# WeChatCV/WeDetect

Measured on AMD Instinct MI355X. Metric: images/s at 640x640 (WeDetect-Base image tower + 80-class similarity + top-k/NMS), higher is better.
Workload: dtype f32-equivalent: fp32 operands carried as fp16 hi+lo pairs, 3 fp16-MFMA passes per product, fp32 accumulate (fp16x3); similarity GEMM, dwconv, LN, post-process native f32

## Files before the change

### wedetect_amd/build.py

```python
from __future__ import annotations

import os
import subprocess
import sys

HERE = os.path.dirname(os.path.abspath(__file__))
ROOT = os.path.dirname(HERE)
CSRC = os.path.join(HERE, "csrc")
LIB = os.path.join(HERE, "libwedetect_hip.so")
SOURCES = ["abi.hip", "conv_gemm.hip", "similarity_grouped.hip", "split_gemm.hip", "split_gemm_pre.hip", "split_gemm_p8.hip", "split_gemm_p4.hip", "split_gemm_conv.hip", "split_gemm_conv3.hip", "split_gemm_mlp.hip", "split_gemm_mlpw.hip", "probe.hip", "stem.hip", "elementwise.hip", "preprocess.hip", "text.hip", "bricks.hip", "evaluate.hip", "det_eval.hip", "postprocess.hip"]
HIPCC = os.environ.get("HIPCC", "/opt/rocm/bin/hipcc")
FLAGS = ["--offload-arch=gfx950", "-O3", "-std=c++17", "-fPIC", "-Wall", "-Wno-unused-function", "-Wno-inline-asm",
         "-I", os.path.join(ROOT, "include"), "-I", CSRC]
for _d in os.environ.get("WD_EXTRA_DEFINES", "").split():
    FLAGS.append("-D" + _d)
if os.environ.get("WD_DEBUG_ABLATIONS") == "1":
    FLAGS.append("-DWD_DEBUG_ABLATIONS")


def _headers():
    return [os.path.join(CSRC, f) for f in os.listdir(CSRC) if f.endswith(".h")] + [os.path.join(ROOT, "include", "wedetect_hip.h")]


def source_hash() -> str:
    import hashlib
    h = hashlib.sha256()
    files = sorted(os.path.join(CSRC, f) for f in os.listdir(CSRC) if f.endswith((".hip", ".h")))
    for f in files + [os.path.join(ROOT, "include", "wedetect_hip.h")]:
        h.update(os.path.basename(f).encode())
        h.update(open(f, "rb").read())
    return h.hexdigest()


NO_SCRATCH = {"stem.hip": ["stem_fused_kernel"], "split_gemm_mlpw.hip": ["fused_mlp_wide_kernel"],
              "split_gemm_mlp.hip": ["fused_mlp128_kernel"], "split_gemm_p8.hip": ["split_gemm_p8_kernel"],
              "split_gemm_p4.hip": ["split_gemm_p4_kernel"], "split_gemm_conv.hip": ["split_conv_pp_kernel"],
              "split_gemm_conv3.hip": ["split_conv3_kernel", "split_conv3w_kernel"],
              "split_gemm_pre.hip": ["split_gemm_pingpong_kernel", "split_gemm_glds_kernel"],
              "elementwise.hip": ["dwconv7_dma_kernel", "dwconv7_ln_reg4_dma_kernel"],
              "similarity_grouped.hip": ["similarity_grouped_kernel"]}
ASM_VMEM_SOURCES = {"split_gemm_mlpw.hip": ["fused_mlp_wide_kernel"], "split_gemm_mlp.hip": [], "split_gemm_p8.hip": [],
                    "split_gemm_p4.hip": [], "split_gemm_pre.hip": [], "split_gemm_conv.hip": [], "split_gemm_conv3.hip": [], "stem.hip": [], "elementwise.hip": [], "similarity_grouped.hip": []}


ASM_DS_READ_SOURCES = {"split_gemm_conv3.hip": ["split_conv3w_kernel"]}


def check_isa(src: str, verbose: bool = True) -> None:
    asm = _obj(src).replace(".o", ".s")
    cmd = [HIPCC, *[f for f in FLAGS if f != "-fPIC"], "-S", "--cuda-device-only", os.path.join(CSRC, src), "-o", asm]
    subprocess.check_call(cmd, stderr=subprocess.DEVNULL)
    scripts = os.path.join(ROOT, "scripts")
    r = subprocess.run([sys.executable, os.path.join(scripts, "check_sgpr_vmem_hazard.py"), asm], capture_output=True, text=True)
    if r.returncode != 0:
        raise RuntimeError(f"SGPR -> VMEM hazard in the ISA of {src}:\n{r.stdout[-2000:]}")
    syms = ASM_VMEM_SOURCES[src]
    if syms:
        r = subprocess.run([sys.executable, os.path.join(scripts, "check_asm_loads.py"), asm, *syms], capture_output=True, text=True)
        if r.returncode != 0:
            raise RuntimeError(f"pending asm load touched in the ISA of {src}:\n{r.stdout[-2000:]}")
    if src in ASM_DS_READ_SOURCES:
        r = subprocess.run([sys.executable, os.path.join(scripts, "check_asm_ds_reads.py"), asm, *ASM_DS_READ_SOURCES[src]], capture_output=True, text=True)
        if r.returncode != 0:
            raise RuntimeError(f"pending asm ds_read touched in the ISA of {src}:\n{r.stdout[-2000:]}")
    if src in NO_SCRATCH:
        import re
        meta = open(asm).read()
        meta = meta[meta.index("amdhsa.kernels"):] if "amdhsa.kernels" in meta else ""
        seen = set()
        for blk in meta.split("- .agpr_count")[1:]:
            name = re.search(r"\.name:\s+(\S+)", blk).group(1)
            scratch = int(re.search(r"\.private_segment_fixed_size:\s+(\d+)", blk).group(1))
            for k in NO_SCRATCH[src]:
                if k in name:
                    seen.add(k)
                    if scratch != 0:
                        raise RuntimeError(f"{src}: kernel {name} uses {scratch} bytes of scratch — its counted vmcnt waits assume none")
        missing = [k for k in NO_SCRATCH[src] if k not in seen]
        if missing:
            raise RuntimeError(f"{src}: NO_SCRATCH names no kernel of this source: {missing}")
    os.remove(asm)
    if verbose:
        print(f"ISA checks passed: {src}", flush=True)


def _obj(src: str) -> str:
    return os.path.join(CSRC, src.replace(".hip", ".o"))


def _obj_stale(src: str) -> bool:
    obj = _obj(src)
    if not os.path.exists(obj):
        return True
    t = os.path.getmtime(obj)
    return any(os.path.getmtime(d) > t for d in [os.path.join(CSRC, src)] + _headers())


def _stale() -> bool:
    if not os.path.exists(LIB):
        return True
    t = os.path.getmtime(LIB)
    return any(_obj_stale(s) or os.path.getmtime(_obj(s)) > t for s in SOURCES)


def build(force: bool = False, verbose: bool = True) -> str:
    if not force and not _stale():
        return LIB
    procs = []
    for src in SOURCES:
        if not force and not _obj_stale(src):
            continue
        cmd = [HIPCC, *FLAGS, "-c", os.path.join(CSRC, src), "-o", _obj(src)]
        if verbose:
            print(" ".join(cmd), flush=True)
        procs.append((src, subprocess.Popen(cmd)))
    import concurrent.futures as cf
    with cf.ThreadPoolExecutor(max_workers=4) as ex:
        checks = [ex.submit(check_isa, src, verbose) for src, _ in procs if src in ASM_VMEM_SOURCES]
        for src, p in procs:
            if p.wait() != 0:
                raise RuntimeError(f"hipcc failed on {src}")
        for c in checks:
            c.result()
    cmd = [HIPCC, "--offload-arch=gfx950", "-shared", "-fPIC", *[_obj(s) for s in SOURCES], "-o", LIB]
    if verbose:
        print(" ".join(cmd), flush=True)
    subprocess.check_call(cmd)
    return LIB


if __name__ == "__main__":
    print(build(force="--force" in sys.argv))
```

### wedetect_amd/csrc/split_gemm_mlpw.hip

```cpp
#include <stdlib.h>
#include "split_epi_oct.h"
#include "split_mlp_epi.h"

namespace {

template <int C>
struct MW {
  static constexpr int H = 4 * C, BM = 128, HC = 128, NCH = H / HC;
  static constexpr int KT = 64, NKT = C / KT;
  static constexpr int XSLOT = BM * 256, NSLOT = 3;
  static constexpr int HOFF = NSLOT * XSLOT;
  static constexpr int LDS = HOFF + BM * 512;
  static constexpr int TN2 = C / 128;
  static constexpr int S1 = C / 16, S2 = H / 16;
  static_assert(C % 128 == 0 && NKT >= 2 && LDS <= 160 * 1024, "shape");
  static_assert(4 * 32 * EPI_LDT * 4 <= HOFF, "the epilogue patches reuse the ring");
};

struct MwArgs {
  const unsigned char* a;
  const unsigned char* w1;
  const unsigned char* w2;
  const float* b1;
  const float* b2;
  float* x;
  unsigned* range_flag;
  int m;
  float unscale1, unscale2, hid_scale;
  unsigned* flag;
  float* park;
  int nblk;
  const float* ln_stats;
  const float* ln_u;
};

#define MW_OPAQUE(p) asm volatile("" : "+s"(p))
template <bool SAFE>
__device__ __forceinline__ void mw_dma(unsigned lds_addr, unsigned voff, const unsigned char* base) {
  if constexpr (SAFE)
    asm volatile("s_mov_b32 m0, %0\n\ts_nop 4\n\tglobal_load_lds_dwordx4 %1, %2" ::"s"(lds_addr), "v"(voff), "s"(base) : "memory", "m0");
  else
    asm volatile("s_mov_b32 m0, %0\n\ts_nop 0\n\tglobal_load_lds_dwordx4 %1, %2" ::"s"(lds_addr), "v"(voff), "s"(base) : "memory", "m0");
}

#ifdef MW_EXPERIMENT_LGKM
#define MW_LGKM0 "s_waitcnt lgkmcnt(0)"
#else
#define MW_LGKM0 ""
#endif
#define MW_BARRIER()                          \
  do {                                        \
    __builtin_amdgcn_sched_barrier(0);        \
    asm volatile(MW_LGKM0 ::: "memory");      \
    __builtin_amdgcn_s_barrier();             \
    asm volatile("" ::: "memory");            \
    __builtin_amdgcn_sched_barrier(0);        \
  } while (0)

template <bool SAFE>
__device__ __forceinline__ void mw_wload(h8& hi, h8& lo, unsigned lane16, const unsigned char* base) {
  if constexpr (SAFE)
    asm volatile("s_nop 4\n\tglobal_load_dwordx4 %0, %2, %3\n\tglobal_load_dwordx4 %1, %2, %3 offset:1024"
                 : "=&v"(hi), "=&v"(lo) : "v"(lane16), "s"(base) : "memory");
  else
    asm volatile("global_load_dwordx4 %0, %2, %3\n\tglobal_load_dwordx4 %1, %2, %3 offset:1024"
                 : "=&v"(hi), "=&v"(lo) : "v"(lane16), "s"(base) : "memory");
}
template <bool SAFE>
__device__ __forceinline__ void mw_bload(f32x4& d, unsigned voff, const float* base) {
  if constexpr (SAFE)
    asm volatile("s_nop 4\n\tglobal_load_dwordx4 %0, %1, %2" : "=&v"(d) : "v"(voff), "s"(base) : "memory");
  else
    asm volatile("global_load_dwordx4 %0, %1, %2" : "=&v"(d) : "v"(voff), "s"(base) : "memory");
}
#define MW_WAIT8_(N, A0, A1, A2, A3, A4, A5, A6, A7) \
  asm volatile("s_waitcnt vmcnt(" #N ")" : "+v"(A0), "+v"(A1), "+v"(A2), "+v"(A3), "+v"(A4), "+v"(A5), "+v"(A6), "+v"(A7) :: "memory")
#ifdef MW_EXPERIMENT_ALL0
#define MW_WAIT8(N, ...) MW_WAIT8_(0, __VA_ARGS__)
#else
#define MW_WAIT8(N, ...) MW_WAIT8_(N, __VA_ARGS__)
#endif

template <int C, int ABL = 0, bool PERSIST = false, bool FOLD = false>
__global__ void __launch_bounds__(256) fused_mlp_wide_kernel(const MwArgs q) {
  using P = MW<C>;
  constexpr int TN2 = P::TN2, NKT = P::NKT;
  static_assert(NKT % 2 == 0 && NKT >= 4, "K tiles alternate between two W1 fragment buffers");
  extern __shared__ __attribute__((aligned(16))) unsigned char smem_raw[];
  const int t = threadIdx.x, lane = t & 63;
  const int wave = __builtin_amdgcn_readfirstlane(t >> 6);
  int first_blk, seg_o, last_blk, seg_e;
  if (PERSIST) {
    const int b = blockIdx.x, xcd = b & 7, slot = b >> 3, per = gridDim.x >> 3;
    const long long t0 = (long long)q.nblk * xcd / 8, t1 = (long long)q.nblk * (xcd + 1) / 8;
    const long long units = (t1 - t0) * P::NCH;
    const long long u0 = t0 * P::NCH + units * slot / per, u1 = t0 * P::NCH + units * (slot + 1) / per;
    first_blk = (int)(u0 / P::NCH); seg_o = (int)(u0 - (long long)first_blk * P::NCH);
    last_blk = (int)(u1 / P::NCH); seg_e = (int)(u1 - (long long)last_blk * P::NCH);
  } else {
    int tile = blockIdx.x;
    const int nwg = gridDim.x, xcd = tile & 7, idx = tile >> 3;
    const int qq = nwg >> 3, r = nwg & 7;
    tile = (xcd < r ? xcd * (qq + 1) : r * (qq + 1) + (xcd - r) * qq) + idx;
    first_blk = tile; seg_o = 0; last_blk = tile + 1; seg_e = 0;
  }
  const int has_head = seg_e > 0, has_tail = seg_o > 0;
  const int full0 = first_blk + has_tail, nfull = last_blk - full0;
  const int nseg = has_head + nfull + has_tail;
  unsigned lds0 = (unsigned)(size_t)(__attribute__((address_space(3))) unsigned char*)smem_raw;

  unsigned la[4];
#pragma unroll
  for (int c = 0; c < 4; ++c) la[c] = (unsigned)(lane >> 4) * (unsigned)(C * 4) + (unsigned)((((lane & 15) ^ (4 * c + (lane >> 4))) & 15) << 4);
  const unsigned char* arow = q.a;
  auto issue_x = [&](int kt, int slot) {
    if (ABL & 2) return;
#pragma unroll
    for (int i = 0; i < 8; ++i) {
      const int g = wave * 8 + i;
      mw_dma<PERSIST>(lds0 + slot * P::XSLOT + g * 1024, la[i & 3], arow + (size_t)(4 * g) * (C * 4) + kt * 256);
    }
  };

  const int r = lane & 31, hsel = lane >> 5, f = r & 15;
  const int xb = r * 256 + (((2 * hsel) ^ f) << 4);
  const int hb = r * 512 + (((2 * hsel) ^ f) << 4);
  const unsigned char* hbuf = smem_raw + P::HOFF;

  const unsigned lane16 = (unsigned)lane * 16u;
  const unsigned char* w1w_ = q.w1 + (size_t)wave * (P::S1 * 2048);
  const unsigned char* w2w_ = q.w2 + (size_t)(TN2 * wave) * (P::S2 * 2048);
  const unsigned char *w1w = w1w_, *w2w = w2w_;
  const unsigned bvoff = (unsigned)hsel * 16u;
  const float* b1p = q.b1 + wave * 32;
  const float* u1p = FOLD ? q.ln_u + wave * 32 : nullptr;

  using I0 = std::integral_constant<int, 0>;
  using I1 = std::integral_constant<int, 1>;

  for (int sg = 0; sg < nseg; ++sg) {
  const bool is_head = has_head && sg == 0;
  const bool is_tail = has_tail && sg == nseg - 1;
  const int blk = is_head ? last_blk : (is_tail ? first_blk : full0 + sg - has_head);
  const int c0 = is_tail ? seg_o : 0, c1 = is_head ? seg_e : P::NCH;
  const int m0 = blk * P::BM;
  arow = q.a + (size_t)m0 * (C * 4);
  MW_BARRIER();

  f32x16 out[4][TN2];
  if (PERSIST && is_tail) {
    const int prev = blockIdx.x - 8;
    if (t == 0) {
      while (__hip_atomic_load(q.flag + prev, __ATOMIC_RELAXED, __HIP_MEMORY_SCOPE_AGENT) != 1u) __builtin_amdgcn_s_sleep(8);
      __builtin_amdgcn_fence(__ATOMIC_ACQUIRE, "agent");
    }
    __syncthreads();
    const unsigned char* sb = reinterpret_cast<const unsigned char*>(q.park) + (size_t)prev * (4 * TN2 * 4 * 4096);
    const unsigned toff = (unsigned)t * 16u;
#pragma unroll
    for (int i = 0; i < 4; ++i) {
      f32x4 v[TN2][4];
#pragma unroll
      for (int jn = 0; jn < TN2; ++jn)
#pragma unroll
        for (int g = 0; g < 4; ++g) {
          MW_OPAQUE(sb);
          v[jn][g] = *reinterpret_cast<const f32x4*>(sb + toff);
          sb += 4096;
        }
#pragma unroll
      for (int jn = 0; jn < TN2; ++jn)
#pragma unroll
        for (int g = 0; g < 4; ++g) {
          out[i][jn][4 * g] = v[jn][g][0]; out[i][jn][4 * g + 1] = v[jn][g][1]; out[i][jn][4 * g + 2] = v[jn][g][2]; out[i][jn][4 * g + 3] = v[jn][g][3];
        }
      __builtin_amdgcn_sched_barrier(0);
#pragma unroll
      for (int jn = 0; jn < TN2; ++jn) asm volatile("" : "+a"(out[i][jn]));
      __builtin_amdgcn_sched_barrier(0);
    }
    asm volatile("s_waitcnt vmcnt(0)" ::: "memory");
    __syncthreads();
    if (t == 0) __hip_atomic_store(q.flag + prev, 0u, __ATOMIC_RELAXED, __HIP_MEMORY_SCOPE_AGENT);
  } else {
#pragma unroll
    for (int i = 0; i < 4; ++i)
#pragma unroll
      for (int jn = 0; jn < TN2; ++jn)
#pragma unroll
        for (int e = 0; e < 16; ++e) out[i][jn][e] = 0.0f;
  }

  h8 wh[2][4], wl[2][4];
  h8 vh[2][TN2], vl[2][TN2];
  f32x4 bq[4];
  f32x4 uq[4] = {};
  typedef float f32x2_ __attribute__((ext_vector_type(2)));
  f32x2_ st[4] = {};

  auto load_w1_tile = [&](int j, int kt, int buf) {
    if ((ABL & 8) && (j > c0 || kt > 1)) return;
    const unsigned char* b = w1w + (size_t)(4 * j) * (P::S1 * 2048) + kt * 8192;
#pragma unroll
    for (int s = 0; s < 4; ++s) mw_wload<PERSIST>(wh[buf][s], wl[buf][s], lane16, b + s * 2048);
  };
  auto load_w2_step = [&](int S, int buf) {
    if ((ABL & 8) && S > 1) return;
    const unsigned char* b = w2w + (size_t)S * 2048;
#pragma unroll
    for (int jn = 0; jn < TN2; ++jn) mw_wload<PERSIST>(vh[buf][jn], vl[buf][jn], lane16, b + (size_t)jn * (P::S2 * 2048));
  };
  auto load_bias = [&](int j) {
    const float* b = b1p + j * P::HC;
#pragma unroll
    for (int g = 0; g < 4; ++g) mw_bload<PERSIST>(bq[g], bvoff, b + 8 * g);
    if constexpr (FOLD) {
      const float* u = u1p + j * P::HC;
#pragma unroll
      for (int g = 0; g < 4; ++g) mw_bload<PERSIST>(uq[g], bvoff, u + 8 * g);
    }
  };

  MW_OPAQUE(arow); MW_OPAQUE(w1w); MW_OPAQUE(w2w); MW_OPAQUE(b1p); MW_OPAQUE(lds0);
  issue_x(0, 0);
  issue_x(1, 1);
  load_w1_tile(c0, 0, 0);
  load_w1_tile(c0, 1, 1);
  load_bias(c0);
  if constexpr (FOLD) {
    const float* sp = q.ln_stats + 2 * (size_t)m0;
    MW_OPAQUE(sp);
#pragma unroll
    for (int i = 0; i < 4; ++i) {
      const unsigned so = (unsigned)(32 * i + r) * 8u;
      if constexpr (PERSIST) asm volatile("s_nop 4\n\tglobal_load_dwordx2 %0, %1, %2" : "=&v"(st[i]) : "v"(so), "s"(sp) : "memory");
      else asm volatile("global_load_dwordx2 %0, %1, %2" : "=&v"(st[i]) : "v"(so), "s"(sp) : "memory");
    }
    asm volatile("s_waitcnt vmcnt(0)" : "+v"(st[0]), "+v"(st[1]), "+v"(st[2]), "+v"(st[3]) :: "memory");
  } else {
    asm volatile("s_waitcnt vmcnt(0)" ::: "memory");
  }

  for (int j = c0; j < c1; ++j) {
    const int jn1 = j + 1 < c1 ? j + 1 : j;
    MW_OPAQUE(arow); MW_OPAQUE(w1w); MW_OPAQUE(w2w); MW_OPAQUE(b1p); MW_OPAQUE(lds0);
    f32x16 g1[4];
#pragma unroll
    for (int i = 0; i < 4; ++i)
#pragma unroll
      for (int e = 0; e < 16; ++e) g1[i][e] = 0.0f;

    auto ktile = [&](auto kt_c, auto buf_c, int slot) {
      constexpr int KT_ = decltype(kt_c)::value, BUF = decltype(buf_c)::value;
      if (!(ABL & 2)) {
#ifdef MW_EXPERIMENT_TILE_WAIT
        MW_WAIT8(MW_EXPERIMENT_TILE_WAIT, wh[BUF][0], wl[BUF][0], wh[BUF][1], wl[BUF][1], wh[BUF][2], wl[BUF][2], wh[BUF][3], wl[BUF][3]);
#else
        if constexpr (KT_ == 0 && TN2 == 2 && FOLD) MW_WAIT8(20, wh[BUF][0], wl[BUF][0], wh[BUF][1], wl[BUF][1], wh[BUF][2], wl[BUF][2], wh[BUF][3], wl[BUF][3]);
        else if constexpr (KT_ == 0 && TN2 == 2) MW_WAIT8(16, wh[BUF][0], wl[BUF][0], wh[BUF][1], wl[BUF][1], wh[BUF][2], wl[BUF][2], wh[BUF][3], wl[BUF][3]);
        else if constexpr (KT_ <= 1 && FOLD) MW_WAIT8(24, wh[BUF][0], wl[BUF][0], wh[BUF][1], wl[BUF][1], wh[BUF][2], wl[BUF][2], wh[BUF][3], wl[BUF][3]);
        else if constexpr (KT_ <= 1) MW_WAIT8(20, wh[BUF][0], wl[BUF][0], wh[BUF][1], wl[BUF][1], wh[BUF][2], wl[BUF][2], wh[BUF][3], wl[BUF][3]);
        else if constexpr (KT_ == NKT - 1) MW_WAIT8(8, wh[BUF][0], wl[BUF][0], wh[BUF][1], wl[BUF][1], wh[BUF][2], wl[BUF][2], wh[BUF][3], wl[BUF][3]);
        else MW_WAIT8(16, wh[BUF][0], wl[BUF][0], wh[BUF][1], wl[BUF][1], wh[BUF][2], wl[BUF][2], wh[BUF][3], wl[BUF][3]);
#endif
      }
      if (!(ABL & 4)) MW_BARRIER();
      {
        int s2 = slot + 2;
        if (s2 >= P::NSLOT) s2 -= P::NSLOT;
        issue_x(KT_ + 2 < NKT ? KT_ + 2 : KT_ + 2 - NKT, s2);
      }
      const unsigned char* xs = smem_raw + slot * P::XSLOT;
      const unsigned char* wnext = w1w + (size_t)(4 * j) * (P::S1 * 2048) + (KT_ + 2) * 8192;
      h8 xh[2][4], xl[2][4];
      auto read_x = [&](int ks, h8 (&fh)[4], h8 (&fl)[4]) {
#pragma unroll
        for (int i = 0; i < 4; ++i) {
          fh[i] = *reinterpret_cast<const h8*>(xs + i * 8192 + (xb ^ (ks * 64)));
          fl[i] = *reinterpret_cast<const h8*>(xs + i * 8192 + (xb ^ (ks * 64 + 16)));
        }
      };
      read_x(0, xh[0], xl[0]);
      __builtin_amdgcn_sched_barrier(0);
#pragma unroll
      for (int ks = 0; ks < 4; ++ks) {
        const int cb = ks & 1;
        if (ks < 3) read_x(ks + 1, xh[cb ^ 1], xl[cb ^ 1]);
#pragma unroll
        for (int i = 0; i < 4; ++i) g1[i] = __builtin_amdgcn_mfma_f32_32x32x16_f16(wl[BUF][ks], xh[cb][i], g1[i], 0, 0, 0);
#pragma unroll
        for (int i = 0; i < 4; ++i) g1[i] = __builtin_amdgcn_mfma_f32_32x32x16_f16(wh[BUF][ks], xl[cb][i], g1[i], 0, 0, 0);
#pragma unroll
        for (int i = 0; i < 4; ++i) g1[i] = __builtin_amdgcn_mfma_f32_32x32x16_f16(wh[BUF][ks], xh[cb][i], g1[i], 0, 0, 0);
        if (ks < 3) {
#pragma unroll
          for (int u = 0; u < 8; ++u) {
            __builtin_amdgcn_sched_group_barrier(0x008, 1, 0);
            __builtin_amdgcn_sched_group_barrier(0x100, 1, 0);
          }
          __builtin_amdgcn_sched_group_barrier(0x008, 4, 0);
        }
        __builtin_amdgcn_sched_barrier(0);
        if constexpr (KT_ + 2 < NKT) {
          if (!(ABL & 8)) mw_wload<PERSIST>(wh[BUF][ks], wl[BUF][ks], lane16, wnext + ks * 2048);
        }
      }
    };
    {
      int slot = 0;
      slot = ((j - c0) * (NKT % P::NSLOT)) % P::NSLOT;
      auto adv = [&]() { slot = slot + 1 == P::NSLOT ? 0 : slot + 1; };
      ktile(std::integral_constant<int, 0>{}, I0{}, slot); adv();
      ktile(std::integral_constant<int, 1>{}, I1{}, slot); adv();
      ktile(std::integral_constant<int, 2>{}, I0{}, slot); adv();
      ktile(std::integral_constant<int, 3>{}, I1{}, slot); adv();
      if constexpr (NKT == 8) {
        ktile(std::integral_constant<int, 4>{}, I0{}, slot); adv();
        ktile(std::integral_constant<int, 5>{}, I1{}, slot); adv();
        ktile(std::integral_constant<int, 6>{}, I0{}, slot); adv();
        ktile(std::integral_constant<int, 7>{}, I1{}, slot); adv();
      }
    }

    load_w2_step(8 * j, 0);
    load_w2_step(8 * j + 1, 1);
#ifdef MW_EXPERIMENT_ALL0
    asm volatile("s_waitcnt vmcnt(0)" : "+v"(bq[0]), "+v"(bq[1]), "+v"(bq[2]), "+v"(bq[3]) :: "memory");
#else
    asm volatile("s_waitcnt vmcnt(48)" : "+v"(bq[0]), "+v"(bq[1]), "+v"(bq[2]), "+v"(bq[3]) :: "memory");
#endif
    if constexpr (FOLD) asm volatile("" : "+v"(uq[0]), "+v"(uq[1]), "+v"(uq[2]), "+v"(uq[3]));

#pragma unroll
    for (int i = 0; i < 4; ++i) {
      u32x2 hi[4], lo[4];
#pragma unroll
      for (int g = 0; g < 4; ++g) {
        if (ABL & 1) {
          hi[g] = u32x2{__builtin_bit_cast(unsigned, g1[i][4 * g]), __builtin_bit_cast(unsigned, g1[i][4 * g + 1])};
          lo[g] = u32x2{__builtin_bit_cast(unsigned, g1[i][4 * g + 2]), __builtin_bit_cast(unsigned, g1[i][4 * g + 3])};
        } else {
          const f32x4 v = {g1[i][4 * g], g1[i][4 * g + 1], g1[i][4 * g + 2], g1[i][4 * g + 3]};
          f32x4 o;
#pragma unroll
          for (int e = 0; e < 4; ++e) {
            if constexpr (FOLD) o[e] = wd_gelu(fmaf(st[i][1], fmaf(-st[i][0], uq[g][e], v[e] * q.unscale1), bq[g][e]));
            else o[e] = wd_gelu(fmaf(v[e], q.unscale1, bq[g][e]));
          }
          if (q.hid_scale != 1.0f) o = o * q.hid_scale;
          split4(o, hi[g], lo[g]);
        }
      }
#pragma unroll
      for (int s = 0; s < 2; ++s) {
        h8 fh8, fl8;
        mc_epi_swap(hi, lo, s, fh8, fl8);
        const int grp = 4 * wave + 2 * s + hsel;
        unsigned char* hp = smem_raw + P::HOFF + (32 * i + r) * 512;
        *reinterpret_cast<h8*>(hp + (((2 * grp) ^ f) << 4)) = fh8;
        *reinterpret_cast<h8*>(hp + (((2 * grp + 1) ^ f) << 4)) = fl8;
      }
    }
    asm volatile("s_waitcnt lgkmcnt(0)" ::: "memory");
    MW_BARRIER();

    h8 hh[2][4], hl[2][4];
    auto read_h = [&](int ks, h8 (&fh)[4], h8 (&fl)[4]) {
#pragma unroll
      for (int i = 0; i < 4; ++i) {
        fh[i] = *reinterpret_cast<const h8*>(hbuf + i * 16384 + (hb ^ (ks * 64)));
        fl[i] = *reinterpret_cast<const h8*>(hbuf + i * 16384 + (hb ^ (ks * 64 + 16)));
      }
    };
    auto g2step = [&](auto ks_c, auto buf_c) {
      constexpr int KS = decltype(ks_c)::value, BUF = decltype(buf_c)::value;
      static_assert(TN2 == 4 || TN2 == 2, "wait operand lists");
      if constexpr (TN2 == 4) {
#define MW_W2WAIT(N) MW_WAIT8(N, vh[BUF][0], vl[BUF][0], vh[BUF][1], vl[BUF][1], vh[BUF][2], vl[BUF][2], vh[BUF][3], vl[BUF][3])
        if constexpr (KS <= 4) MW_W2WAIT(8); else if constexpr (KS == 5) MW_W2WAIT(16); else if constexpr (KS == 6) MW_W2WAIT(24); else if constexpr (FOLD) MW_W2WAIT(16); else MW_W2WAIT(12);
#undef MW_W2WAIT
      } else {
#ifdef MW_EXPERIMENT_ALL0
#define MW_W2WAIT(N) asm volatile("s_waitcnt vmcnt(0)" : "+v"(vh[BUF][0]), "+v"(vl[BUF][0]), "+v"(vh[BUF][1]), "+v"(vl[BUF][1]) :: "memory")
#else
#define MW_W2WAIT(N) asm volatile("s_waitcnt vmcnt(" #N ")" : "+v"(vh[BUF][0]), "+v"(vl[BUF][0]), "+v"(vh[BUF][1]), "+v"(vl[BUF][1]) :: "memory")
#endif
        if constexpr (KS <= 4) MW_W2WAIT(4); else if constexpr (KS == 5) MW_W2WAIT(12); else if constexpr (KS == 6) MW_W2WAIT(20); else if constexpr (FOLD) MW_W2WAIT(16); else MW_W2WAIT(12);
#undef MW_W2WAIT
      }
      if constexpr (KS == 0) {
        read_h(0, hh[0], hl[0]);
        __builtin_amdgcn_sched_barrier(0);
      }
      if constexpr (KS < 7) read_h(KS + 1, hh[BUF ^ 1], hl[BUF ^ 1]);
#pragma unroll
      for (int i = 0; i < 4; ++i)
#pragma unroll
        for (int jn = 0; jn < TN2; ++jn) out[i][jn] = __builtin_amdgcn_mfma_f32_32x32x16_f16(vl[BUF][jn], hh[BUF][i], out[i][jn], 0, 0, 0);
#pragma unroll
      for (int i = 0; i < 4; ++i)
#pragma unroll
        for (int jn = 0; jn < TN2; ++jn) out[i][jn] = __builtin_amdgcn_mfma_f32_32x32x16_f16(vh[BUF][jn], hl[BUF][i], out[i][jn], 0, 0, 0);
#pragma unroll
      for (int i = 0; i < 4; ++i)
#pragma unroll
        for (int jn = 0; jn < TN2; ++jn) out[i][jn] = __builtin_amdgcn_mfma_f32_32x32x16_f16(vh[BUF][jn], hh[BUF][i], out[i][jn], 0, 0, 0);
      if constexpr (KS < 7) {
#pragma unroll
        for (int u = 0; u < 8; ++u) {
          __builtin_amdgcn_sched_group_barrier(0x008, 1, 0);
          __builtin_amdgcn_sched_group_barrier(0x100, 1, 0);
        }
        __builtin_amdgcn_sched_group_barrier(0x008, 12 * TN2 - 8, 0);
      }
      __builtin_amdgcn_sched_barrier(0);
      if constexpr (KS < 6) load_w2_step(8 * j + KS + 2, BUF);
      if constexpr (KS == 4) load_w1_tile(jn1, 0, 0);
      if constexpr (KS == 5) load_w1_tile(jn1, 1, 1);
      if constexpr (KS == 6) load_bias(jn1);
    };
    g2step(std::integral_constant<int, 0>{}, I0{});
    g2step(std::integral_constant<int, 1>{}, I1{});
    g2step(std::integral_constant<int, 2>{}, I0{});
    g2step(std::integral_constant<int, 3>{}, I1{});
    g2step(std::integral_constant<int, 4>{}, I0{});
    g2step(std::integral_constant<int, 5>{}, I1{});
    g2step(std::integral_constant<int, 6>{}, I0{});
    g2step(std::integral_constant<int, 7>{}, I1{});
  }
  MW_WAIT8(0, wh[0][0], wl[0][0], wh[0][1], wl[0][1], wh[0][2], wl[0][2], wh[0][3], wl[0][3]);
  asm volatile("" : "+v"(wh[1][0]), "+v"(wl[1][0]), "+v"(wh[1][1]), "+v"(wl[1][1]), "+v"(wh[1][2]), "+v"(wl[1][2]), "+v"(wh[1][3]), "+v"(wl[1][3]));
  asm volatile("" : "+v"(bq[0]), "+v"(bq[1]), "+v"(bq[2]), "+v"(bq[3]));
  if constexpr (FOLD) asm volatile("" : "+v"(uq[0]), "+v"(uq[1]), "+v"(uq[2]), "+v"(uq[3]));
#pragma unroll
  for (int jn = 0; jn < TN2; ++jn) asm volatile("" : "+v"(vh[0][jn]), "+v"(vl[0][jn]), "+v"(vh[1][jn]), "+v"(vl[1][jn]));
  MW_BARRIER();

  if (PERSIST && is_head) {
    unsigned char* sb = reinterpret_cast<unsigned char*>(q.park) + (size_t)blockIdx.x * (4 * TN2 * 4 * 4096);
    const unsigned toff = (unsigned)t * 16u;
#pragma unroll
    for (int i = 0; i < 4; ++i)
#pragma unroll
      for (int jn = 0; jn < TN2; ++jn)
#pragma unroll
        for (int g = 0; g < 4; ++g) {
          MW_OPAQUE(sb);
          *reinterpret_cast<f32x4*>(sb + toff) = f32x4{out[i][jn][4 * g], out[i][jn][4 * g + 1], out[i][jn][4 * g + 2], out[i][jn][4 * g + 3]};
          sb += 4096;
        }
    asm volatile("s_waitcnt vmcnt(0)" ::: "memory");
    __syncthreads();
    if (t == 0) {
      __builtin_amdgcn_fence(__ATOMIC_RELEASE, "agent");
      asm volatile("s_waitcnt vmcnt(0)" ::: "memory");
      __hip_atomic_store(q.flag + blockIdx.x, 1u, __ATOMIC_RELAXED, __HIP_MEMORY_SCOPE_AGENT);
    }
    continue;
  }
  WdConvGemm pe{};
  pe.bias = q.b2; pe.res = q.x; pe.c = q.x; pe.m = q.m; pe.n = C; pe.ldc = C; pe.ldres = C;
  pe.act = WD_ACT_NONE; pe.out_mode = WD_OUT_ROWS; pe.res_alpha = 1.0f; pe.out_scale = 1.0f; pe.range_flag = q.range_flag;
  float* patch = reinterpret_cast<float*>(smem_raw) + wave * 32 * EPI_LDT;
  const int nw = wave * (C / 4);
#pragma unroll
  for (int i = 0; i < 4; ++i) {
    f32x16 row[1][TN2];
#pragma unroll
    for (int jn = 0; jn < TN2; ++jn) row[0][jn] = out[i][jn];
    EpiOctOperands<1, TN2> ops;
    ops.load(pe, m0 + 32 * i, nw, lane);
    EpiOctWalk<0, 1, TN2, WD_ACT_NONE, false, false>::run(pe, q.unscale2, m0 + 32 * i, nw, lane, row, patch, ops);
  }
  }
}

int mw_workgroups() {
  static int n[64] = {};
  int dev = 0;
  if (hipGetDevice(&dev) != hipSuccess) return -1;
  int& slot = n[dev & 63];
  if (!slot) {
    hipDeviceProp_t prop;
    if (hipGetDeviceProperties(&prop, dev) != hipSuccess) return -1;
    slot = prop.multiProcessorCount / 8 * 8;
  }
  return slot;
}

template <int C, int ABL = 0, bool FOLD = false>
int launch_mlp_wide(MwArgs q, hipStream_t st, float* ws, long long ws_floats) {
  using P = MW<C>;
  const int nblk = q.m / P::BM;
  q.nblk = nblk;
  const int wgs = mw_workgroups();
  constexpr bool PERSIST_BUILT = C != 512;
  const bool persist = PERSIST_BUILT && ws != nullptr && wgs > 0 && nblk / 8 >= wgs / 8 && nblk > wgs &&
                       ws_floats >= 1024 + (long long)wgs * (4 * P::TN2 * 4 * 256 * 4);
  if constexpr (PERSIST_BUILT) if (persist) {
    q.flag = reinterpret_cast<unsigned*>(ws);
    q.park = ws + 1024;
    static WdAttrOnce attr;
    if (wd_set_max_lds(attr, reinterpret_cast<const void*>(fused_mlp_wide_kernel<C, ABL, true, FOLD>), P::LDS) != WD_OK) return WD_ERR_LAUNCH;
    WD_LAUNCH_GEMM((fused_mlp_wide_kernel<C, ABL, true, FOLD>), dim3((unsigned)wgs), dim3(256), P::LDS, st, q);
    return wd_launch_status();
  }
  static WdAttrOnce attr;
  if (wd_set_max_lds(attr, reinterpret_cast<const void*>(fused_mlp_wide_kernel<C, ABL, false, FOLD>), P::LDS) != WD_OK) return WD_ERR_LAUNCH;
  WD_LAUNCH_GEMM((fused_mlp_wide_kernel<C, ABL, false, FOLD>), dim3((unsigned)nblk), dim3(256), P::LDS, st, q);
  return wd_launch_status();
}

}

extern "C" int wd_mlp_fused_wide(const void* a_split, int64_t rows, int32_t c, int32_t hidden, const void* w1_frag,
                                 float w1_unscale, const float* b1, const void* w2_frag, float w2_unscale, const float* b2,
                                 float* x, float hid_scale, uint32_t* range_flag, void* workspace, int64_t workspace_bytes,
                                 void* stream) {
  if (workspace && (!wd_aligned16(workspace) || workspace_bytes < 0)) return WD_ERR_BAD_ARG;
  if (!a_split || !w1_frag || !w2_frag || !b1 || !b2 || !x) return WD_ERR_BAD_ARG;
  if ((c != 256 && c != 512) || hidden != 4 * c) return WD_ERR_UNSUPPORTED;
  if (rows <= 0 || rows % 128 || rows / 128 > 0x7fffffffLL) return WD_ERR_UNSUPPORTED;
  if (!wd_aligned16(a_split) || !wd_aligned16(w1_frag) || !wd_aligned16(w2_frag) || !wd_aligned16(b1) || !wd_aligned16(b2) ||
      !wd_aligned16(x))
    return WD_ERR_BAD_ARG;
  if (!(w1_unscale > 0.f) || !(w2_unscale > 0.f) || !(hid_scale > 0.f)) return WD_ERR_BAD_ARG;
  MwArgs q{static_cast<const unsigned char*>(a_split), static_cast<const unsigned char*>(w1_frag),
           static_cast<const unsigned char*>(w2_frag), b1, b2, x, range_flag, (int)rows, w1_unscale, w2_unscale, hid_scale,
           nullptr, nullptr, 0, nullptr, nullptr};
  float* ws = static_cast<float*>(workspace);
  const long long wsf = workspace ? workspace_bytes / 4 : 0;
  hipStream_t st = static_cast<hipStream_t>(stream);
#ifdef WD_DEBUG_ABLATIONS
  if (const char* e = getenv("WD_MLPW_ABL")) {
    if (c != 512) return WD_ERR_UNSUPPORTED;
    switch (atoi(e)) {
      case 1: return launch_mlp_wide<512, 1>(q, st, ws, wsf);
      case 2: return launch_mlp_wide<512, 2>(q, st, ws, wsf);
      case 4: return launch_mlp_wide<512, 4>(q, st, ws, wsf);
      case 6: return launch_mlp_wide<512, 6>(q, st, ws, wsf);
      case 7: return launch_mlp_wide<512, 7>(q, st, ws, wsf);
      case 8: return launch_mlp_wide<512, 8>(q, st, ws, wsf);
      case 14: return launch_mlp_wide<512, 14>(q, st, ws, wsf);
      case 15: return launch_mlp_wide<512, 15>(q, st, ws, wsf);
      default: break;
    }
  }
#endif
  return c == 512 ? launch_mlp_wide<512>(q, st, ws, wsf) : launch_mlp_wide<256>(q, st, ws, wsf);
}

extern "C" int wd_mlp_fused_wide_ln(const void* d_split, int64_t rows, int32_t c, int32_t hidden, const void* w1g_frag,
                                    float w1_unscale, const float* v, const float* u, const float* ln_stats, const void* w2_frag,
                                    float w2_unscale, const float* b2, float* x, float hid_scale, uint32_t* range_flag,
                                    void* workspace, int64_t workspace_bytes, void* stream) {
  if (workspace && (!wd_aligned16(workspace) || workspace_bytes < 0)) return WD_ERR_BAD_ARG;
  if (!d_split || !w1g_frag || !w2_frag || !v || !u || !ln_stats || !b2 || !x) return WD_ERR_BAD_ARG;
  if (c != 256 || hidden != 4 * c) return WD_ERR_UNSUPPORTED;
  if (rows <= 0 || rows % 128 || rows / 128 > 0x7fffffffLL) return WD_ERR_UNSUPPORTED;
  if (!wd_aligned16(d_split) || !wd_aligned16(w1g_frag) || !wd_aligned16(w2_frag) || !wd_aligned16(v) || !wd_aligned16(u) ||
      !wd_aligned16(b2) || !wd_aligned16(x) || (reinterpret_cast<uintptr_t>(ln_stats) & 7u))
    return WD_ERR_BAD_ARG;
  if (!(w1_unscale > 0.f) || !(w2_unscale > 0.f) || !(hid_scale > 0.f)) return WD_ERR_BAD_ARG;
  MwArgs q{static_cast<const unsigned char*>(d_split), static_cast<const unsigned char*>(w1g_frag),
           static_cast<const unsigned char*>(w2_frag), v, b2, x, range_flag, (int)rows, w1_unscale, w2_unscale, hid_scale,
           nullptr, nullptr, 0, ln_stats, u};
  return launch_mlp_wide<256, 0, true>(q, static_cast<hipStream_t>(stream), static_cast<float*>(workspace), workspace ? workspace_bytes / 4 : 0);
}
```

Baseline: 980.2.

## Add resident-panel 64-row fused MLP kernel for C=256 stages

Adds a dedicated fused MLP kernel for C=256 that keeps the whole 64-row input panel resident in LDS, double-buffers the hidden chunk, and overlaps the GELU epilogue of one hidden chunk with the next chunk's first GEMM. The C=256 path now always launches this kernel with one workgroup per 64 rows instead of the 128-row ring/persistent kernel. Smaller row tiles mean more workgroups and finer load balance, at the cost of reloading weights more often per row. It relies on hand-counted vmcnt waits, so any change in the load order could break correctness.

```diff
diff --git a/wedetect_amd/build.py b/wedetect_amd/build.py
--- a/wedetect_amd/build.py
+++ b/wedetect_amd/build.py
@@ -32,14 +32,14 @@
     return h.hexdigest()
 
 
-NO_SCRATCH = {"stem.hip": ["stem_fused_kernel"], "split_gemm_mlpw.hip": ["fused_mlp_wide_kernel"],
+NO_SCRATCH = {"stem.hip": ["stem_fused_kernel"], "split_gemm_mlpw.hip": ["fused_mlp_wide_kernel", "fused_mlp_res256_kernel"],
               "split_gemm_mlp.hip": ["fused_mlp128_kernel"], "split_gemm_p8.hip": ["split_gemm_p8_kernel"],
               "split_gemm_p4.hip": ["split_gemm_p4_kernel"], "split_gemm_conv.hip": ["split_conv_pp_kernel"],
               "split_gemm_conv3.hip": ["split_conv3_kernel", "split_conv3w_kernel"],
               "split_gemm_pre.hip": ["split_gemm_pingpong_kernel", "split_gemm_glds_kernel"],
               "elementwise.hip": ["dwconv7_dma_kernel", "dwconv7_ln_reg4_dma_kernel"],
               "similarity_grouped.hip": ["similarity_grouped_kernel"]}
-ASM_VMEM_SOURCES = {"split_gemm_mlpw.hip": ["fused_mlp_wide_kernel"], "split_gemm_mlp.hip": [], "split_gemm_p8.hip": [],
+ASM_VMEM_SOURCES = {"split_gemm_mlpw.hip": ["fused_mlp_wide_kernel", "fused_mlp_res256_kernel"], "split_gemm_mlp.hip": [], "split_gemm_p8.hip": [],
                     "split_gemm_p4.hip": [], "split_gemm_pre.hip": [], "split_gemm_conv.hip": [], "split_gemm_conv3.hip": [], "stem.hip": [], "elementwise.hip": [], "similarity_grouped.hip": []}
 
 
diff --git a/wedetect_amd/csrc/split_gemm_mlpw.hip b/wedetect_amd/csrc/split_gemm_mlpw.hip
--- a/wedetect_amd/csrc/split_gemm_mlpw.hip
+++ b/wedetect_amd/csrc/split_gemm_mlpw.hip
@@ -475,6 +475,351 @@
   }
 }
 
+struct MR {
+  static constexpr int C = 256, H = 4 * C, BM = 64, HC = 128, NCH = H / HC;
+  static constexpr int NKT = C / 64, XT = BM * 256;
+  static constexpr int HOFF = NKT * XT;
+  static constexpr int HB = BM * 512;
+  static constexpr int LDS = HOFF + 2 * HB;
+  static constexpr int TN2 = C / 128, S1 = C / 16, S2 = H / 16;
+  static_assert(LDS <= 160 * 1024 && 4 * 32 * EPI_LDT * 4 <= HOFF, "the epilogue patches reuse the panel");
+};
+
+#ifndef MW_RES_ABL
+#define MW_RES_ABL 0
+#endif
+
+template <bool FOLD>
+__device__ __forceinline__ void mr_epi_elem(float acc, float b, float u, float mean, float rstd, float unscale1, float hid_scale,
+                                            _Float16& h, _Float16& l) {
+#pragma clang fp contract(off)
+  if (MW_RES_ABL & 1) { h = (_Float16)acc; l = (_Float16)b; return; }
+  const float pre = FOLD ? fmaf(rstd, fmaf(-mean, u, acc * unscale1), b) : fmaf(acc, unscale1, b);
+  float o = wd_gelu(pre) * hid_scale;
+  asm("" : "+v"(o));
+  h = (_Float16)o;
+  l = (_Float16)(o - (float)h);
+}
+
+template <bool FOLD>
+__global__ void __launch_bounds__(256) fused_mlp_res256_kernel(const MwArgs q) {
+  using P = MR;
+  constexpr int C = P::C, TN2 = P::TN2, NKT = P::NKT;
+  static_assert(NKT == 4 && TN2 == 2, "wait counts");
+  extern __shared__ __attribute__((aligned(16))) unsigned char smem_raw[];
+  const int t = threadIdx.x, lane = t & 63;
+  const int wave = __builtin_amdgcn_readfirstlane(t >> 6);
+  int tile = blockIdx.x;
+  {
+    const int nwg = gridDim.x, xcd = tile & 7, idx = tile >> 3;
+    const int qq = nwg >> 3, rr = nwg & 7;
+    tile = (xcd < rr ? xcd * (qq + 1) : rr * (qq + 1) + (xcd - rr) * qq) + idx;
+  }
+  const int m0 = tile * P::BM;
+  unsigned lds0 = (unsigned)(size_t)(__attribute__((address_space(3))) unsigned char*)smem_raw;
+
+  unsigned la[4];
+#pragma unroll
+  for (int c = 0; c < 4; ++c) la[c] = (unsigned)(lane >> 4) * (unsigned)(C * 4) + (unsigned)((((lane & 15) ^ (4 * c + (lane >> 4))) & 15) << 4);
+  const unsigned char* arow = q.a + (size_t)m0 * (C * 4);
+
+  const int r = lane & 31, hsel = lane >> 5, f = r & 15;
+  const int xb = r * 256 + (((2 * hsel) ^ f) << 4);
+  const int hb = r * 512 + (((2 * hsel) ^ f) << 4);
+
+  const unsigned lane16 = (unsigned)lane * 16u;
+  const unsigned char* w1w = q.w1 + (size_t)wave * (P::S1 * 2048);
+  const unsigned char* w2w = q.w2 + (size_t)(TN2 * wave) * (P::S2 * 2048);
+  const unsigned bvoff = (unsigned)hsel * 16u;
+  const float* b1p = q.b1 + wave * 32;
+  const float* u1p = FOLD ? q.ln_u + wave * 32 : nullptr;
+
+  using I0 = std::integral_constant<int, 0>;
+  using I1 = std::integral_constant<int, 1>;
+  using I2 = std::integral_constant<int, 2>;
+  using I3 = std::integral_constant<int, 3>;
+  using I4 = std::integral_constant<int, 4>;
+  using I5 = std::integral_constant<int, 5>;
+  using I6 = std::integral_constant<int, 6>;
+  using I7 = std::integral_constant<int, 7>;
+
+  f32x16 out[2][TN2];
+#pragma unroll
+  for (int i = 0; i < 2; ++i)
+#pragma unroll
+    for (int jn = 0; jn < TN2; ++jn)
+#pragma unroll
+      for (int e = 0; e < 16; ++e) out[i][jn][e] = 0.0f;
+
+  h8 wh[2][4], wl[2][4];
+  h8 vh[2][TN2], vl[2][TN2];
+  f32x4 bq[4];
+  f32x4 uq[4] = {};
+  typedef float f32x2_ __attribute__((ext_vector_type(2)));
+  f32x2_ st[2] = {};
+
+  bool in_loop = false;
+  auto w1_tile_off = [](int T) { return (size_t)(T >> 2) * (4 * P::S1 * 2048) + (size_t)(T & 3) * 8192; };
+  auto load_w1_tile = [&](int T, int buf) {
+    const unsigned char* b = w1w + w1_tile_off(T);
+#pragma unroll
+    for (int s = 0; s < 4; ++s) mw_wload<false>(wh[buf][s], wl[buf][s], lane16, b + s * 2048);
+  };
+  auto load_w2_step = [&](int S, int buf) {
+    if ((MW_RES_ABL & 8) && in_loop) return;
+    const unsigned char* b = w2w + (size_t)S * 2048;
+#pragma unroll
+    for (int jn = 0; jn < TN2; ++jn) mw_wload<false>(vh[buf][jn], vl[buf][jn], lane16, b + (size_t)jn * (P::S2 * 2048));
+  };
+  auto load_bias = [&](int j) {
+    const float* b = b1p + j * P::HC;
+#pragma unroll
+    for (int g = 0; g < 4; ++g) mw_bload<false>(bq[g], bvoff, b + 8 * g);
+    if constexpr (FOLD) {
+      const float* u = u1p + j * P::HC;
+#pragma unroll
+      for (int g = 0; g < 4; ++g) mw_bload<false>(uq[g], bvoff, u + 8 * g);
+    }
+  };
+
+  _Float16 eh[4], el[4];
+  u32x2 ghi[4], glo[4];
+  auto gelu_piece = [&](int n, const f32x16 (&src)[2], unsigned char* hbuf) {
+    typedef _Float16 ph2 __attribute__((ext_vector_type(2)));
+    const int i = n >> 3, g = (n >> 1) & 3, e0 = 2 * (n & 1);
+#pragma unroll
+    for (int e = e0; e < e0 + 2; ++e)
+      mr_epi_elem<FOLD>(src[i][4 * g + e], bq[g][e], uq[g][e], st[i][0], st[i][1], q.unscale1, q.hid_scale, eh[e], el[e]);
+    if (n & 1) {
+      ghi[g] = u32x2{__builtin_bit_cast(unsigned, ph2{eh[0], eh[1]}), __builtin_bit_cast(unsigned, ph2{eh[2], eh[3]})};
+      glo[g] = u32x2{__builtin_bit_cast(unsigned, ph2{el[0], el[1]}), __builtin_bit_cast(unsigned, ph2{el[2], el[3]})};
+    }
+    if ((n & 7) == 7) {
+#pragma unroll
+      for (int s = 0; s < 2; ++s) {
+        h8 fh8, fl8;
+        mc_epi_swap(ghi, glo, s, fh8, fl8);
+        const int grp = 4 * wave + 2 * s + hsel;
+        unsigned char* hp = hbuf + (32 * i + r) * 512;
+        *reinterpret_cast<h8*>(hp + (((2 * grp) ^ f) << 4)) = fh8;
+        *reinterpret_cast<h8*>(hp + (((2 * grp + 1) ^ f) << 4)) = fl8;
+      }
+    }
+  };
+
+  auto gemm1 = [&](auto ovl_c, int jg, f32x16 (&acc)[2], const f32x16 (&src)[2], unsigned char* hbuf) {
+    constexpr bool OVL = decltype(ovl_c)::value;
+#pragma unroll
+    for (int i = 0; i < 2; ++i)
+#pragma unroll
+      for (int e = 0; e < 16; ++e) acc[i][e] = 0.0f;
+    auto ktile = [&](auto kt_c, auto buf_c) {
+      constexpr int KT_ = decltype(kt_c)::value, BUF = decltype(buf_c)::value;
+      if constexpr (KT_ == 0) {
+        MW_WAIT8(28, wh[BUF][0], wl[BUF][0], wh[BUF][1], wl[BUF][1], wh[BUF][2], wl[BUF][2], wh[BUF][3], wl[BUF][3]);
+        asm volatile("" : "+v"(bq[0]), "+v"(bq[1]), "+v"(bq[2]), "+v"(bq[3]));
+        if constexpr (FOLD) asm volatile("" : "+v"(uq[0]), "+v"(uq[1]), "+v"(uq[2]), "+v"(uq[3]));
+      } else if constexpr (KT_ == 1 && FOLD) MW_WAIT8(48, wh[BUF][0], wl[BUF][0], wh[BUF][1], wl[BUF][1], wh[BUF][2], wl[BUF][2], wh[BUF][3], wl[BUF][3]);
+      else if constexpr (KT_ == 1) MW_WAIT8(44, wh[BUF][0], wl[BUF][0], wh[BUF][1], wl[BUF][1], wh[BUF][2], wl[BUF][2], wh[BUF][3], wl[BUF][3]);
+      else MW_WAIT8(8, wh[BUF][0], wl[BUF][0], wh[BUF][1], wl[BUF][1], wh[BUF][2], wl[BUF][2], wh[BUF][3], wl[BUF][3]);
+      const unsigned char* xs = smem_raw + KT_ * P::XT;
+      int tn = 4 * jg + KT_ + 2;
+      if (tn > 4 * P::NCH - 1) tn -= 4;
+      const unsigned char* wnext = w1w + w1_tile_off(tn);
+      h8 xh[2][2], xl[2][2];
+      auto read_x = [&](int ks, h8 (&fh)[2], h8 (&fl)[2]) {
+#pragma unroll
+        for (int i = 0; i < 2; ++i) {
+          fh[i] = *reinterpret_cast<const h8*>(xs + i * 8192 + (xb ^ (ks * 64)));
+          fl[i] = *reinterpret_cast<const h8*>(xs + i * 8192 + (xb ^ (ks * 64 + 16)));
+        }
+      };
+      read_x(0, xh[0], xl[0]);
+      __builtin_amdgcn_sched_barrier(0);
+#pragma unroll
+      for (int ks = 0; ks < 4; ++ks) {
+        const int cb = ks & 1;
+        if (ks < 3 && !(MW_RES_ABL & 16)) read_x(ks + 1, xh[cb ^ 1], xl[cb ^ 1]);
+#pragma unroll
+        for (int i = 0; i < 2; ++i) acc[i] = __builtin_amdgcn_mfma_f32_32x32x16_f16(wl[BUF][ks], xh[cb][i], acc[i], 0, 0, 0);
+#pragma unroll
+        for (int i = 0; i < 2; ++i) acc[i] = __builtin_amdgcn_mfma_f32_32x32x16_f16(wh[BUF][ks], xl[cb][i], acc[i], 0, 0, 0);
+#pragma unroll
+        for (int i = 0; i < 2; ++i) acc[i] = __builtin_amdgcn_mfma_f32_32x32x16_f16(wh[BUF][ks], xh[cb][i], acc[i], 0, 0, 0);
+        if constexpr (OVL) gelu_piece(4 * KT_ + ks, src, hbuf);
+#pragma unroll
+        for (int u = 0; u < 6; ++u) {
+          __builtin_amdgcn_sched_group_barrier(0x008, 1, 0);
+          if (u < 4 && ks < 3) __builtin_amdgcn_sched_group_barrier(0x100, 1, 0);
+          if constexpr (OVL) __builtin_amdgcn_sched_group_barrier(0x002, 6, 0);
+        }
+        __builtin_amdgcn_sched_barrier(0);
+        if (!((MW_RES_ABL & 8) && in_loop)) mw_wload<false>(wh[BUF][ks], wl[BUF][ks], lane16, wnext + ks * 2048);
+      }
+    };
+    ktile(I0{}, I0{});
+    ktile(I1{}, I1{});
+    ktile(I2{}, I0{});
+    ktile(I3{}, I1{});
+  };
+
+  auto gemm2 = [&](auto tail_c, int j, const unsigned char* hbuf) {
+    constexpr bool TAIL = decltype(tail_c)::value;
+    const int jn1 = j + 1 < P::NCH ? j + 1 : j;
+    h8 hh[2][2], hl[2][2];
+    auto read_h = [&](int ks, h8 (&fh)[2], h8 (&fl)[2]) {
+#pragma unroll
+      for (int i = 0; i < 2; ++i) {
+        fh[i] = *reinterpret_cast<const h8*>(hbuf + i * 16384 + (hb ^ (ks * 64)));
+        fl[i] = *reinterpret_cast<const h8*>(hbuf + i * 16384 + (hb ^ (ks * 64 + 16)));
+      }
+    };
+    auto g2step = [&](auto ks_c, auto buf_c) {
+      constexpr int KS = decltype(ks_c)::value, BUF = decltype(buf_c)::value;
+#ifdef MW_EXPERIMENT_ALL0
+#define MW_W2WAIT(N) asm volatile("s_waitcnt vmcnt(0)" : "+v"(vh[BUF][0]), "+v"(vl[BUF][0]), "+v"(vh[BUF][1]), "+v"(vl[BUF][1]) :: "memory")
+#else
+#define MW_W2WAIT(N) asm volatile("s_waitcnt vmcnt(" #N ")" : "+v"(vh[BUF][0]), "+v"(vl[BUF][0]), "+v"(vh[BUF][1]), "+v"(vl[BUF][1]) :: "memory")
+#endif
+      if constexpr (KS == 0 && TAIL) MW_W2WAIT(4);
+      else if constexpr (KS == 0) MW_W2WAIT(36);
+      else if constexpr (KS == 1 && TAIL && FOLD) MW_W2WAIT(12);
+      else if constexpr (KS == 1 && TAIL) MW_W2WAIT(8);
+      else if constexpr (KS == 1 && FOLD) MW_W2WAIT(44);
+      else if constexpr (KS == 1) MW_W2WAIT(40);
+      else if constexpr (KS == 2 && FOLD) MW_W2WAIT(12);
+      else if constexpr (KS == 2) MW_W2WAIT(8);
+      else MW_W2WAIT(4);
+#undef MW_W2WAIT
+      if constexpr (KS == 0) {
+        read_h(0, hh[0], hl[0]);
+        __builtin_amdgcn_sched_barrier(0);
+      }
+      if constexpr (KS < 7 && !(MW_RES_ABL & 16)) read_h(KS + 1, hh[BUF ^ 1], hl[BUF ^ 1]);
+#pragma unroll
+      for (int i = 0; i < 2; ++i)
+#pragma unroll
+        for (int jn = 0; jn < TN2; ++jn) out[i][jn] = __builtin_amdgcn_mfma_f32_32x32x16_f16(vl[BUF][jn], hh[BUF][i], out[i][jn], 0, 0, 0);
+#pragma unroll
+      for (int i = 0; i < 2; ++i)
+#pragma unroll
+        for (int jn = 0; jn < TN2; ++jn) out[i][jn] = __builtin_amdgcn_mfma_f32_32x32x16_f16(vh[BUF][jn], hl[BUF][i], out[i][jn], 0, 0, 0);
+#pragma unroll
+      for (int i = 0; i < 2; ++i)
+#pragma unroll
+        for (int jn = 0; jn < TN2; ++jn) out[i][jn] = __builtin_amdgcn_mfma_f32_32x32x16_f16(vh[BUF][jn], hh[BUF][i], out[i][jn], 0, 0, 0);
+      if constexpr (KS < 7) {
+#pragma unroll
+        for (int u = 0; u < 4; ++u) {
+          __builtin_amdgcn_sched_group_barrier(0x008, 1, 0);
+          __builtin_amdgcn_sched_group_barrier(0x100, 1, 0);
+        }
+        __builtin_amdgcn_sched_group_barrier(0x008, 6 * TN2 - 4, 0);
+      }
+      __builtin_amdgcn_sched_barrier(0);
+      if constexpr (KS < 6) load_w2_step(8 * j + KS + 2, BUF);
+      else load_w2_step(8 * jn1 + KS - 6, BUF);
+      if constexpr (KS == 0) load_bias(jn1);
+    };
+    g2step(I0{}, I0{});
+    g2step(I1{}, I1{});
+    g2step(I2{}, I0{});
+    g2step(I3{}, I1{});
+    g2step(I4{}, I0{});
+    g2step(I5{}, I1{});
+    g2step(I6{}, I0{});
+    g2step(I7{}, I1{});
+  };
+
+  MW_OPAQUE(arow); MW_OPAQUE(w1w); MW_OPAQUE(w2w); MW_OPAQUE(b1p); MW_OPAQUE(lds0);
+#pragma unroll
+  for (int kt = 0; kt < NKT; ++kt)
+#pragma unroll
+    for (int i = 0; i < 4; ++i) {
+      const int g = wave * 4 + i;
+      mw_dma<false>(lds0 + kt * P::XT + g * 1024, la[i], arow + (size_t)(4 * g) * (C * 4) + kt * 256);
+    }
+  load_w1_tile(0, 0);
+  load_w1_tile(1, 1);
+  load_bias(0);
+  load_w2_step(0, 0);
+  load_w2_step(1, 1);
+  if constexpr (FOLD) {
+    const float* sp = q.ln_stats + 2 * (size_t)m0;
+    MW_OPAQUE(sp);
+#pragma unroll
+    for (int i = 0; i < 2; ++i) {
+      const unsigned so = (unsigned)(32 * i + r) * 8u;
+      asm volatile("global_load_dwordx2 %0, %1, %2" : "=&v"(st[i]) : "v"(so), "s"(sp) : "memory");
+    }
+    asm volatile("s_waitcnt vmcnt(0)" : "+v"(st[0]), "+v"(st[1]) :: "memory");
+  } else {
+    asm volatile("s_waitcnt vmcnt(0)" ::: "memory");
+  }
+#pragma unroll
+  for (int jn = 0; jn < TN2; ++jn) asm volatile("" : "+v"(vh[0][jn]), "+v"(vl[0][jn]), "+v"(vh[1][jn]), "+v"(vl[1][jn]));
+  MW_BARRIER();
+
+  f32x16 g1c[2], g1n[2];
+  gemm1(std::false_type{}, 0, g1c, g1c, smem_raw);
+  MW_WAIT8(0, wh[0][0], wl[0][0], wh[0][1], wl[0][1], wh[0][2], wl[0][2], wh[0][3], wl[0][3]);
+  asm volatile("" : "+v"(wh[1][0]), "+v"(wl[1][0]), "+v"(wh[1][1]), "+v"(wl[1][1]), "+v"(wh[1][2]), "+v"(wl[1][2]), "+v"(wh[1][3]), "+v"(wl[1][3]));
+
+#pragma unroll 1
+  for (int j = 0; j < P::NCH - 1; ++j) {
+    in_loop = true;
+    MW_OPAQUE(w1w); MW_OPAQUE(w2w); MW_OPAQUE(b1p);
+    unsigned char* hbuf = smem_raw + P::HOFF + (j & 1) * P::HB;
+    gemm1(std::true_type{}, j + 1, g1n, g1c, hbuf);
+    asm volatile("s_waitcnt lgkmcnt(0)" ::: "memory");
+    if (!(MW_RES_ABL & 4)) MW_BARRIER();
+    gemm2(std::false_type{}, j, hbuf);
+#pragma unroll
+    for (int i = 0; i < 2; ++i) g1c[i] = g1n[i];
+  }
+  {
+    constexpr int j = P::NCH - 1;
+    unsigned char* hbuf = smem_raw + P::HOFF + (j & 1) * P::HB;
+    asm volatile("s_waitcnt vmcnt(8)" : "+v"(bq[0]), "+v"(bq[1]), "+v"(bq[2]), "+v"(bq[3]) :: "memory");
+    if constexpr (FOLD) asm volatile("" : "+v"(uq[0]), "+v"(uq[1]), "+v"(uq[2]), "+v"(uq[3]));
+#pragma unroll
+    for (int n = 0; n < 16; ++n) gelu_piece(n, g1c, hbuf);
+    asm volatile("s_waitcnt lgkmcnt(0)" ::: "memory");
+    if (!(MW_RES_ABL & 4)) MW_BARRIER();
+    gemm2(std::true_type{}, j, hbuf);
+  }
+  MW_WAIT8(0, wh[0][0], wl[0][0], wh[0][1], wl[0][1], wh[0][2], wl[0][2], wh[0][3], wl[0][3]);
+  asm volatile("" : "+v"(wh[1][0]), "+v"(wl[1][0]), "+v"(wh[1][1]), "+v"(wl[1][1]), "+v"(wh[1][2]), "+v"(wl[1][2]), "+v"(wh[1][3]), "+v"(wl[1][3]));
+  asm volatile("" : "+v"(bq[0]), "+v"(bq[1]), "+v"(bq[2]), "+v"(bq[3]));
+  if constexpr (FOLD) asm volatile("" : "+v"(uq[0]), "+v"(uq[1]), "+v"(uq[2]), "+v"(uq[3]));
+#pragma unroll
+  for (int jn = 0; jn < TN2; ++jn) asm volatile("" : "+v"(vh[0][jn]), "+v"(vl[0][jn]), "+v"(vh[1][jn]), "+v"(vl[1][jn]));
+  MW_BARRIER();
+
+  WdConvGemm pe{};
+  pe.bias = q.b2; pe.res = q.x; pe.c = q.x; pe.m = q.m; pe.n = C; pe.ldc = C; pe.ldres = C;
+  pe.act = WD_ACT_NONE; pe.out_mode = WD_OUT_ROWS; pe.res_alpha = 1.0f; pe.out_scale = 1.0f; pe.range_flag = q.range_flag;
+  float* patch = reinterpret_cast<float*>(smem_raw) + wave * 32 * EPI_LDT;
+  const int nw = wave * (C / 4);
+#pragma unroll
+  for (int i = 0; i < 2; ++i) {
+    f32x16 row[1][TN2];
+#pragma unroll
+    for (int jn = 0; jn < TN2; ++jn) row[0][jn] = out[i][jn];
+    EpiOctOperands<1, TN2> ops;
+    ops.load(pe, m0 + 32 * i, nw, lane);
+    EpiOctWalk<0, 1, TN2, WD_ACT_NONE, false, false>::run(pe, q.unscale2, m0 + 32 * i, nw, lane, row, patch, ops);
+  }
+}
+
+template <bool FOLD>
+int launch_mlp_res256(MwArgs q, hipStream_t st) {
+  static WdAttrOnce attr;
+  if (wd_set_max_lds(attr, reinterpret_cast<const void*>(fused_mlp_res256_kernel<FOLD>), MR::LDS) != WD_OK) return WD_ERR_LAUNCH;
+  WD_LAUNCH_GEMM((fused_mlp_res256_kernel<FOLD>), dim3((unsigned)(q.m / MR::BM)), dim3(256), MR::LDS, st, q);
+  return wd_launch_status();
+}
+
 int mw_workgroups() {
   static int n[64] = {};
   int dev = 0;
@@ -491,6 +836,17 @@
 template <int C, int ABL = 0, bool FOLD = false>
 int launch_mlp_wide(MwArgs q, hipStream_t st, float* ws, long long ws_floats) {
   using P = MW<C>;
+  if constexpr (C == 256 && ABL == 0) {
+#ifdef WD_DEBUG_ABLATIONS
+    static const bool ring256 = getenv("WD_MLPW_RING256") && atoi(getenv("WD_MLPW_RING256")) == 1;
+    if (!ring256)
+#endif
+      return launch_mlp_res256<FOLD>(q, st);
+  }
+#if !defined(WD_DEBUG_ABLATIONS)
+  if constexpr (C == 256) return WD_ERR_UNSUPPORTED; else
+#endif
+  {
   const int nblk = q.m / P::BM;
   q.nblk = nblk;
   const int wgs = mw_workgroups();
@@ -509,6 +865,7 @@
   if (wd_set_max_lds(attr, reinterpret_cast<const void*>(fused_mlp_wide_kernel<C, ABL, false, FOLD>), P::LDS) != WD_OK) return WD_ERR_LAUNCH;
   WD_LAUNCH_GEMM((fused_mlp_wide_kernel<C, ABL, false, FOLD>), dim3((unsigned)nblk), dim3(256), P::LDS, st, q);
   return wd_launch_status();
+  }
 }
 
 }
```

Result: no change. 983.6, median of 6 (+0.4%).
